# robflynnyh/dynamic-asr-eval

Hardware: AMD Instinct MI355X
Metric: audio-sec/s dynamic-eval (fwd+1 adapt step) (higher is better)
Workload: dtype f32; 1 GPU; run_dynamic_eval_full: 1 h Earnings-22-shape recording per step (360000 frames, seq_len 16384, overlap 14336, offline, MADGRAD lr 9e-05, 6 freq masks <=34), SCConformerXL 6x768 V+1=4096 seeded weights; windows_per_recording=169, chains_per_gpu=2, lockstep_group=4, hip_graphs=True, pcie_inclusive=False

## Files before the change

dynamic-asr-eval_amd/csrc/gemm_f32.hip:

```cpp
#include <algorithm>
#include "common.h"
#include <cstdlib>

typedef float f32x16 __attribute__((ext_vector_type(16)));

namespace {

#ifndef DYN_GEMM_BK
#define DYN_GEMM_BK 32
#endif
constexpr int BK = DYN_GEMM_BK;
constexpr int LDK = BK + 4;
constexpr int KV = BK / 4;
constexpr int RP = 256 / KV;
constexpr int NTHREADS = 256;

struct KParams {
    int64_t M, N, K;
    const float* A; int64_t lda, sa1, sa2;
    const float* B; int64_t ldb, sb1, sb2;
    float* C; int64_t ldc, sc1, sc2;
    int64_t cin_delta;
    const float* bias;
    int64_t bs1, bs2;
// ... 4 lines not shown
    float* ws;
    int64_t nbatch;
    int tiles_n;
    int tiles_m;
    int n_major;
    int64_t tiles_per_batch;
    int64_t full_items;
    int tail_f;
    float* tail_ws;
    int epi;
    float* aux;
    int* counters;
    float* colsum;
    float colsum_beta;
    int64_t first_item;
};

__device__ __forceinline__ float epi_value(float alpha, float acc, float beta, const float* cin, float bias) {
    float v = __fmul_rn(alpha, acc);
    if (beta != 0.f) v = __fmaf_rn(beta, *cin, v);
    return __fadd_rn(v, bias);
}

__device__ __forceinline__ float silu_f(float v) { return v * dyn::sigmoidf_(v); }
__device__ __forceinline__ float silu_grad_f(float u) {
    const float sg = dyn::sigmoidf_(u);
    return sg * (1.f + u * (1.f - sg));
}

template <bool KMAJOR, int R>
__device__ __forceinline__ void load_tile_full(const float* __restrict__ base, int64_t ld, int64_t row0, int64_t k0,
                                               float4 (&reg)[(R * BK / 1024)]) {
    const int t = threadIdx.x;
    if (KMAJOR) {
        const float* p = base + (row0 + (t / KV)) * ld + k0 + 4 * (t % KV);
#pragma unroll
        for (int j = 0; j < (R * BK / 1024); ++j) reg[j] = *reinterpret_cast<const float4*>(p + (int64_t)(RP * j) * ld);
    } else {
        constexpr int RV = R / 4;
        constexpr int KSTEP = NTHREADS / RV;
        const float* p = base + (k0 + t / RV) * ld + row0 + 4 * (t % RV);
#pragma unroll
        for (int j = 0; j < (R * BK / 1024); ++j) reg[j] = *reinterpret_cast<const float4*>(p + (int64_t)(KSTEP * j) * ld);
    }
}

// ... 107 lines not shown
        }
        step = KMAJOR ? (int64_t)BK : (int64_t)BK * ld;
    }
    __device__ __forceinline__ void issue(float* tile, int wave) {
#pragma unroll
        for (int j = 0; j < NI; ++j) {
            __builtin_amdgcn_global_load_lds((gbl_void_t*)ptr[j], (lds_void_t*)(tile + (wave * NI + j) * 256), 16, 0, 0);
            ptr[j] += step;
        }
    }
};

template <bool KMAJOR, int R>
__device__ __forceinline__ void read_frag_glds(const float* __restrict__ s, int roff, int i, int h, int c, float (&f)[4]) {
    if (KMAJOR) {
        const float4 v = *reinterpret_cast<const float4*>(&s[(roff + i) * BK + 4 * ((2 * c + h) ^ ((i >> 1) & 7))]);
        f[0] = v.x; f[1] = v.y; f[2] = v.z; f[3] = v.w;
    } else {
#pragma unroll
        for (int q = 0; q < 4; ++q) f[q] = s[(8 * c + 4 * h + q) * R + roff + i];
    }
}

template <bool TA, bool TB, int BM, int BN, bool VEC, bool GLDS, bool GROUPED, int NW = 4>
__device__ __forceinline__ void gemm_tile(const KParams& p, const int64_t bid, float* smem) {
    constexpr bool AK = !TA;
    constexpr bool BKM = TB;
    constexpr int WM = NW / 2;
    constexpr int WTM = BM / (32 * WM), WTN = BN / 64;
    static_assert(NW == 4 || (NW == 8 && GLDS), "the 8-wave tile exists for direct-to-LDS staging only");
    static_assert(!GLDS || (VEC && BK == 32), "direct-to-LDS staging needs 16-B aligned operands and BK = 32");
    constexpr int SA = GLDS ? BM * BK : BM * LDK, SB = GLDS ? BN * BK : BN * LDK;

    const bool is_tail = !GROUPED && bid >= p.full_items;
    int64_t item;
    int sub = 0;
    if (GROUPED) {
        item = bid;
    } else if (!is_tail) {
        const int64_t nwg = p.full_items;
        const int64_t xcd = bid & 7, q = nwg >> 3, r = nwg & 7;
        item = (xcd < r ? xcd * (q + 1) : r * (q + 1) + (xcd - r) * q) + (bid >> 3);
    } else {
        const int64_t t = bid - p.full_items;
        item = p.full_items + t / p.tail_f;
        sub = (int)(t % p.tail_f);
    }
    const int ks = (int)(item % p.splits);
    const int64_t t2 = item / p.splits;
    const int tile = (int)(t2 % p.tiles_per_batch);
    const int zb = (int)(t2 / p.tiles_per_batch);
    const int tm = p.n_major ? tile % p.tiles_m : tile / p.tiles_n;
    const int tn = p.n_major ? tile / p.tiles_m : tile % p.tiles_n;
    const int64_t z1 = zb / p.nb2, z2 = zb % p.nb2;
    const float* A = p.A + z1 * p.sa1 + z2 * p.sa2;
    const float* B = p.B + z1 * p.sb1 + z2 * p.sb2;

    const int64_t m0 = (int64_t)tm * BM, n0 = (int64_t)tn * BN;
    int64_t kbeg = (int64_t)ks * p.kchunk;
    int64_t kend = (kbeg + p.kchunk < p.K) ? kbeg + p.kchunk : p.K;
    if (is_tail) {
        const int64_t kt_all = (kend - kbeg + BK - 1) / BK;
        const int64_t per = (kt_all + p.tail_f - 1) / p.tail_f;
        const int64_t kb2 = kbeg + (int64_t)sub * per * BK;
        const int64_t ke2 = kb2 + per * BK;
        kend = ke2 < kend ? ke2 : kend;
        kbeg = kb2;
    }
    const int nk = kend > kbeg ? (int)((kend - kbeg + BK - 1) / BK) : 0;

    const int lane = threadIdx.x & 63, wave = threadIdx.x >> 6;
    const int i = lane & 31, h = lane >> 5;
    const int wm = wave >> 1, wn = wave & 1;

    f32x16 acc[WTM][WTN];
#pragma unroll
    for (int a = 0; a < WTM; ++a)
#pragma unroll
        for (int b = 0; b < WTN; ++b)
#pragma unroll
            for (int e = 0; e < 16; ++e) acc[a][b][e] = 0.f;

    float4 ra[BM * BK / 1024], rb[BN * BK / 1024];
    const bool interior = VEC && (m0 + BM <= p.M) && (n0 + BN <= p.N);
    auto fetch = [&](int64_t k0) {
        if (interior && k0 + BK <= kend) {
            load_tile_full<AK, BM>(A, p.lda, m0, k0, ra);
            load_tile_full<BKM, BN>(B, p.ldb, n0, k0, rb);
        } else {
            load_tile<AK, BM, VEC>(A, p.lda, m0, p.M, k0, kend, ra);
            load_tile<BKM, BN, VEC>(B, p.ldb, n0, p.N, k0, kend, rb);
        }
    };
    GldsStager<AK, BM, NW> stA;
    GldsStager<BKM, BN, NW> stB;
    if (GLDS) {
        stA.init(A, p.lda, m0, p.M, kbeg, wave, lane);
        stB.init(B, p.ldb, n0, p.N, kbeg, wave, lane);
        if (nk > 0) { stA.issue(smem, wave); stB.issue(smem + SA, wave); }
    } else if (nk > 0) {
        fetch(kbeg);
        store_tile<AK, BM>(smem, ra);
        store_tile<BKM, BN>(smem + SA, rb);
    }
    if (GLDS) asm volatile("s_waitcnt vmcnt(0)" ::: "memory");
    __syncthreads();

    constexpr int NC = BK / 8;
    constexpr int NREADS = (AK ? WTM : 4 * WTM) + (BKM ? WTN : 4 * WTN);
    static_assert(NC % 2 == 0, "the register ping-pong assumes an even number of k-chunks per tile");
    float fa[2][WTM][4], fb[2][WTN][4];
    auto read_chunk = [&](const float* sa, const float* sb, int c, int slot) {
#pragma unroll
        for (int a = 0; a < WTM; ++a) {
            if (GLDS) read_frag_glds<AK, BM>(sa, wm * (BM / WM) + a * 32, i, h, c, fa[slot][a]);
            else read_frag<AK, BM>(sa, wm * (BM / WM) + a * 32, i, h, c, fa[slot][a]);
        }
#pragma unroll
        for (int b = 0; b < WTN; ++b) {
            if (GLDS) read_frag_glds<BKM, BN>(sb, wn * (BN / 2) + b * 32, i, h, c, fb[slot][b]);
            else read_frag<BKM, BN>(sb, wn * (BN / 2) + b * 32, i, h, c, fb[slot][b]);
        }
    };
    float csum[WTM];
#pragma unroll
    for (int a = 0; a < WTM; ++a) csum[a] = 0.f;
    const bool do_colsum = GROUPED && p.colsum != nullptr && tn == 0 && wn == 0;
    auto mfma_chunk = [&](int slot) {
        if (GROUPED && do_colsum) {
#pragma unroll
            for (int a = 0; a < WTM; ++a) csum[a] += (fa[slot][a][0] + fa[slot][a][1]) + (fa[slot][a][2] + fa[slot][a][3]);
        }
#pragma unroll
        for (int s = 0; s < 4; ++s)
#pragma unroll
            for (int a = 0; a < WTM; ++a)
#pragma unroll
                for (int b = 0; b < WTN; ++b)
                    acc[a][b] = __builtin_amdgcn_mfma_f32_32x32x2f32(fa[slot][a][s], fb[slot][b][s], acc[a][b], 0, 0, 0);
    };
    int cur = 0;
    if (nk > 0) read_chunk(smem, smem + SA, 0, 0);
    for (int kt = 0; kt < nk; ++kt) {
        const float* sa = smem + cur * (SA + SB);
// ... 9 lines not shown
        for (int c = 0; c < NC - 1; ++c) {
            read_chunk(sa, sb, c + 1, (c + 1) & 1);
            mfma_chunk(c & 1);
            __builtin_amdgcn_sched_group_barrier(0x100, NREADS, 0);
            __builtin_amdgcn_sched_group_barrier(0x008, 4 * WTM * WTN, 0);
        }
        if (!GLDS && more) {
            store_tile<AK, BM>(da, ra);
            store_tile<BKM, BN>(da + SA, rb);
        }
        if (GLDS) asm volatile("s_waitcnt vmcnt(0)" ::: "memory");
        __syncthreads();
        if (more) read_chunk(da, da + SA, 0, 0);
        mfma_chunk((NC - 1) & 1);
        __builtin_amdgcn_sched_group_barrier(0x100, NREADS, 0);
        __builtin_amdgcn_sched_group_barrier(0x008, 4 * WTM * WTN, 0);
        cur ^= 1;
    }

    if (GROUPED && do_colsum) {
#pragma unroll
        for (int a = 0; a < WTM; ++a) {
            const float tot = csum[a] + __shfl_xor(csum[a], 32);
            const int64_t m = m0 + wm * (BM / WM) + a * 32 + i;
            if (h == 0 && m < p.M) p.colsum[m] = (p.colsum_beta != 0.f ? p.colsum_beta * p.colsum[m] : 0.f) + tot;
        }
    }
    const bool partial = !GROUPED && (is_tail || p.splits > 1);
    if (partial && p.counters == nullptr) {
        if (is_tail) {
            float* W = p.tail_ws + ((item - p.full_items) * p.tail_f + sub) * (int64_t)(BM * BN);
#pragma unroll
            for (int a = 0; a < WTM; ++a)
#pragma unroll
                for (int b = 0; b < WTN; ++b) {
                    float* wp = W + (wm * (BM / WM) + a * 32 + 4 * h) * BN + wn * (BN / 2) + b * 32 + i;
#pragma unroll
                    for (int e = 0; e < 16; ++e) wp[((e & 3) + 8 * (e >> 2)) * BN] = acc[a][b][e];
                }
        } else {
            float* W = p.ws + ((int64_t)ks * p.nbatch + zb) * p.M * p.N;
#pragma unroll
            for (int a = 0; a < WTM; ++a)
#pragma unroll
                for (int b = 0; b < WTN; ++b) {
                    const int64_t col = n0 + wn * (BN / 2) + b * 32 + i;
#pragma unroll
                    for (int e = 0; e < 16; ++e) {
                        const int64_t row = m0 + wm * (BM / WM) + a * 32 + (e & 3) + 8 * (e >> 2) + 4 * h;
                        if (row < p.M && col < p.N) W[row * p.N + col] = acc[a][b][e];
                    }
                }
        }
        return;
    }
    if (partial) {
        const int64_t pt = is_tail ? (item - p.full_items) : t2;
        const int sl = is_tail ? sub : ks;
        const int nsl = is_tail ? p.tail_f : p.splits;
        float* W0 = p.tail_ws + pt * nsl * (int64_t)(BM * BN);
        float* W = W0 + (int64_t)sl * (BM * BN);
#pragma unroll
        for (int a = 0; a < WTM; ++a)
#pragma unroll
            for (int b = 0; b < WTN; ++b) {
                float* wp = W + (wm * (BM / WM) + a * 32 + 4 * h) * BN + wn * (BN / 2) + b * 32 + i;
#pragma unroll
                for (int e = 0; e < 16; ++e) wp[((e & 3) + 8 * (e >> 2)) * BN] = acc[a][b][e];
            }
        __threadfence();
        __syncthreads();
        int* flag = reinterpret_cast<int*>(smem);
        if (threadIdx.x == 0) flag[0] = (atomicAdd(&p.counters[pt], 1) == nsl - 1) ? 1 : 0;
        __syncthreads();
        if (flag[0] == 0) return;
        __threadfence();
#pragma unroll
        for (int a = 0; a < WTM; ++a)
#pragma unroll
            for (int b = 0; b < WTN; ++b) {
                const float* rp = W0 + (wm * (BM / WM) + a * 32 + 4 * h) * BN + wn * (BN / 2) + b * 32 + i;
#pragma unroll
                for (int e = 0; e < 16; ++e) {
                    const float* q = rp + ((e & 3) + 8 * (e >> 2)) * BN;
                    float t = q[0];
                    for (int k = 1; k < nsl; ++k) t += q[(int64_t)k * (BM * BN)];
                    acc[a][b][e] = t;
                }
            }
        if (threadIdx.x == 0) p.counters[pt] = 0;
    }
    if (m0 + BM <= p.M && n0 + BN <= p.N) {
        float* C = p.C + z1 * p.sc1 + z2 * p.sc2;
#pragma unroll
        for (int a = 0; a < WTM; ++a)
#pragma unroll
            for (int b = 0; b < WTN; ++b) {
                const int64_t col = n0 + wn * (BN / 2) + b * 32 + i;
                const float bv = p.bias ? p.bias[z1 * p.bs1 + z2 * p.bs2 + col] : 0.f;
                float* cp = C + (m0 + wm * (BM / WM) + a * 32 + 4 * h) * p.ldc + col;
                if (p.epi != 0) {
                    const int64_t ad = p.aux - p.C;
#pragma unroll
                    for (int e = 0; e < 16; ++e) {
                        float* q2 = cp + (int64_t)((e & 3) + 8 * (e >> 2)) * p.ldc;
                        const float v = epi_value(p.alpha, acc[a][b][e], p.beta, q2 + p.cin_delta, bv);
                        if (p.epi == 1) { if (p.aux) q2[ad] = v; *q2 = silu_f(v); }
                        else *q2 = v * silu_grad_f(q2[ad]);
                    }
                } else if (p.beta != 0.f) {
#pragma unroll
                    for (int e = 0; e < 16; ++e) {
                        float* q2 = cp + (int64_t)((e & 3) + 8 * (e >> 2)) * p.ldc;
                        *q2 = epi_value(p.alpha, acc[a][b][e], p.beta, q2 + p.cin_delta, bv);
                    }
                } else {
#pragma unroll
                    for (int e = 0; e < 16; ++e) cp[(int64_t)((e & 3) + 8 * (e >> 2)) * p.ldc] = epi_value(p.alpha, acc[a][b][e], 0.f, nullptr, bv);
                }
            }
    } else {
        float* C = p.C + z1 * p.sc1 + z2 * p.sc2;
#pragma unroll
        for (int a = 0; a < WTM; ++a)
#pragma unroll
            for (int b = 0; b < WTN; ++b) {
                const int64_t col = n0 + wn * (BN / 2) + b * 32 + i;
                const float bv = (p.bias && col < p.N) ? p.bias[z1 * p.bs1 + z2 * p.bs2 + col] : 0.f;
#pragma unroll
                for (int e = 0; e < 16; ++e) {
                    const int64_t row = m0 + wm * (BM / WM) + a * 32 + (e & 3) + 8 * (e >> 2) + 4 * h;
                    if (row < p.M && col < p.N) {
                        float v = epi_value(p.alpha, acc[a][b][e], p.beta, C + row * p.ldc + col + p.cin_delta, bv);
                        if (p.epi == 1) { if (p.aux) C[row * p.ldc + col + (p.aux - p.C)] = v; v = silu_f(v); }
                        else if (p.epi == 2) v *= silu_grad_f(C[row * p.ldc + col + (p.aux - p.C)]);
                        C[row * p.ldc + col] = v;
                    }
                }
            }
    }
}

#ifndef DYN_GEMM_WAVES_PER_EU
#define DYN_GEMM_WAVES_PER_EU 2
#endif
template <bool TA, bool TB, int BM, int BN, bool VEC, bool GLDS, int NW = 4>
__global__ __launch_bounds__(NW * 64) __attribute__((amdgpu_waves_per_eu(DYN_GEMM_WAVES_PER_EU, 8))) void gemm_f32_kernel(const KParams p) {
    constexpr int SA = GLDS ? BM * BK : BM * LDK, SB = GLDS ? BN * BK : BN * LDK;
    __shared__ __attribute__((aligned(16))) float smem[2 * (SA + SB)];
    gemm_tile<TA, TB, BM, BN, VEC, GLDS, false, NW>(p, (int64_t)blockIdx.x, smem);
}

constexpr int kMaxGroups = 96;
constexpr int kTableChunk = 12;
struct KTableChunk { KParams g[kTableChunk]; };

__global__ void gemm_table_kernel(const KTableChunk chunk, KParams* __restrict__ table, int base, int count) {
    const int t = threadIdx.x;
    if (t < count) table[base + t] = chunk.g[t];
}

template <bool TA, bool TB, int BM, int BN, bool GLDS>
__global__ __launch_bounds__(NTHREADS) void gemm_f32_grouped_kernel(const KParams* __restrict__ table, int n_groups, int64_t total_items) {
    constexpr int SA = GLDS ? BM * BK : BM * LDK, SB = GLDS ? BN * BK : BN * LDK;
    __shared__ __attribute__((aligned(16))) float smem[2 * (SA + SB)];
    const int64_t bid = blockIdx.x;
    const int64_t xcd = bid & 7, q = total_items >> 3, r = total_items & 7;
    const int64_t item = (xcd < r ? xcd * (q + 1) : r * (q + 1) + (xcd - r) * q) + (bid >> 3);
    int lo = 0, hi = n_groups - 1;
    while (lo < hi) {
        const int mid = (lo + hi + 1) >> 1;
        if (table[mid].first_item <= item) lo = mid; else hi = mid - 1;
    }
    const int g = __builtin_amdgcn_readfirstlane(lo);
    const KParams p = table[g];
    gemm_tile<TA, TB, BM, BN, true, GLDS, true>(p, item - p.first_item, smem);
}

__global__ void splitk_reduce_kernel(const KParams p) {
    const int64_t mn = p.M * p.N;
    const int64_t total = mn * p.nbatch;
    for (int64_t idx = (int64_t)blockIdx.x * blockDim.x + threadIdx.x; idx < total;
         idx += (int64_t)gridDim.x * blockDim.x) {
        const int64_t zb = idx / mn, rem = idx % mn;
        const int64_t row = rem / p.N, col = rem % p.N;
        float s = 0.f;
        for (int k = 0; k < p.splits; ++k) s += p.ws[((int64_t)k * p.nbatch + zb) * mn + rem];
        const int64_t z1 = zb / p.nb2, z2 = zb % p.nb2;
        float* C = p.C + z1 * p.sc1 + z2 * p.sc2 + row * p.ldc + col;
        float v = epi_value(p.alpha, s, p.beta, C + p.cin_delta, p.bias ? p.bias[z1 * p.bs1 + z2 * p.bs2 + col] : 0.f);
        if (p.epi == 1) { if (p.aux) C[p.aux - p.C] = v; v = silu_f(v); }
        else if (p.epi == 2) v *= silu_grad_f(C[p.aux - p.C]);
        *C = v;
    }
}

__global__ __launch_bounds__(256) void tail_reduce_kernel(const KParams p, int BM, int BN, int64_t tail_items) {
    const int per_tile = BM * BN / 4;
    const int64_t total = tail_items * per_tile;
// ... 21 lines not shown
            const int64_t col = col0 + j;
            if (col < p.N) {
                float o = epi_value(p.alpha, v[j], p.beta, C + col + p.cin_delta, p.bias ? p.bias[z1 * p.bs1 + z2 * p.bs2 + col] : 0.f);
                if (p.epi == 1) { if (p.aux) C[col + (p.aux - p.C)] = o; o = silu_f(o); }
                else if (p.epi == 2) o *= silu_grad_f(C[col + (p.aux - p.C)]);
                C[col] = o;
            }
        }
    }
}

struct Plan {
    int bm, bn, splits;
    int64_t kchunk;
    int64_t ws_bytes;
    int64_t full_items;
    int64_t tail_items;
    int tail_f;
    int64_t tail_ws_bytes;
};

double tile_eff(int bm, int bn) { return bm == 256 ? 0.84 : (bm == 128 && bn == 128) ? 0.80 : (bm == 64 && bn == 64) ? 0.62 : 0.72; }
int tile_occ(int bm, int bn) { return bm == 256 ? 1 : (bm == 64 && bn == 64) ? 4 : (bm == 128 && bn == 128) ? 2 : 3; }

bool glds_eligible(const dyn_gemm_desc* d) {
    auto al16 = [](const void* q) { return (((uintptr_t)q) & 15) == 0; };
    const bool vec = al16(d->A) && al16(d->B) && (d->lda % 4 == 0) && (d->ldb % 4 == 0) && (d->sa1 % 4 == 0) && (d->sa2 % 4 == 0) &&
                     (d->sb1 % 4 == 0) && (d->sb2 % 4 == 0);
    static const bool allow_glds = [] { const char* e = getenv("DYN_GEMM_GLDS"); return !e || atoi(e) != 0; }();
    const bool ta = d->trans_a != 0, tb = d->trans_b != 0;
    return allow_glds && vec && d->K % BK == 0 && d->K > 0 && (!ta || d->M % 4 == 0) && (tb || d->N % 4 == 0) && (!ta || d->M >= 4) && (tb || d->N >= 4);
}

bool eval_config(const dyn_gemm_desc* d, int bm, int bn, int s, int f_req, Plan* out, double* cost) {
    const int64_t batch = d->nb1 * d->nb2;
    const int64_t ktiles = dyn::cdiv(d->K > 0 ? d->K : 1, BK);
    if (s < 1) s = 1;
    if (s > ktiles) s = (int)ktiles;
    const int64_t tiles = dyn::cdiv(d->M, bm) * dyn::cdiv(d->N, bn);
    const int64_t slots = (int64_t)tile_occ(bm, bn) * 256;
    const int64_t kchunk = dyn::cdiv(ktiles, s) * BK;
    const int s_eff = (int)dyn::cdiv(d->K > 0 ? d->K : 1, kchunk);
    const int64_t items = tiles * batch * s_eff;
    const int64_t rounds = items / slots, rem = items % slots;
    int f = 1;
    if (s_eff == 1 && rem > 0 && f_req != 1) {
// ... 58 lines not shown
            return best;
        }
    }
    const int cand[4][2] = {{128, 128}, {128, 64}, {64, 128}, {64, 64}};
    int split_opts[9] = {1, 2, 3, 4, 6, 8, 12, 16, 24};
    int n_opts = 9;
    if (d->split_k > 0) { split_opts[0] = d->split_k; n_opts = 1; }
    double best_cost = 1e300;
    for (int c = 0; c < 4; ++c) {
        const int bm = cand[c][0], bn = cand[c][1];
        if ((d->M <= 64 && bm == 128) || (d->N <= 64 && bn == 128)) continue;
        for (int so = 0; so < n_opts; ++so) {
            const int s = split_opts[so];
            if (d->split_k == 0 && s > 1 && (d->K / s < 256)) continue;
            Plan pl;
            eval_config(d, bm, bn, s, d->split_k == 0 ? -1 : 1, &pl, &cost);
            if (cost < best_cost) { best_cost = cost; best = pl; }
        }
    }
    return best;
}

template <bool TA, bool TB, int BM, int BN>
void launch_vec(const KParams& kp, bool vec, dim3 grid, hipStream_t st) {
    static const bool allow_glds = [] { const char* e = getenv("DYN_GEMM_GLDS"); return !e || atoi(e) != 0; }();
    const bool glds = allow_glds && vec && kp.K % BK == 0 && kp.K > 0 && (!TA || kp.M % 4 == 0) && (TB || kp.N % 4 == 0) &&
                      (!TA || kp.M >= 4) && (TB || kp.N >= 4);
    if (glds) hipLaunchKernelGGL((gemm_f32_kernel<TA, TB, BM, BN, true, true>), grid, dim3(NTHREADS), 0, st, kp);
    else if (vec) hipLaunchKernelGGL((gemm_f32_kernel<TA, TB, BM, BN, true, false>), grid, dim3(NTHREADS), 0, st, kp);
    else hipLaunchKernelGGL((gemm_f32_kernel<TA, TB, BM, BN, false, false>), grid, dim3(NTHREADS), 0, st, kp);
}

template <bool TA, bool TB>
void launch_tile(const KParams& kp, const Plan& pl, bool vec, dim3 grid, hipStream_t st) {
    if (pl.bm == 256) hipLaunchKernelGGL((gemm_f32_kernel<TA, TB, 256, 128, true, true, 8>), grid, dim3(512), 0, st, kp);
    else if (pl.bm == 128 && pl.bn == 128) launch_vec<TA, TB, 128, 128>(kp, vec, grid, st);
    else if (pl.bm == 128 && pl.bn == 64) launch_vec<TA, TB, 128, 64>(kp, vec, grid, st);
    else if (pl.bm == 64 && pl.bn == 128) launch_vec<TA, TB, 64, 128>(kp, vec, grid, st);
    else launch_vec<TA, TB, 64, 64>(kp, vec, grid, st);
}

}

extern "C" int64_t dyn_gemm_f32_workspace_bytes(const dyn_gemm_desc* d) {
    if (!d || d->M <= 0 || d->N <= 0 || d->nb1 <= 0 || d->nb2 <= 0) return 0;
    const Plan pl = make_plan(d);
    return pl.ws_bytes > pl.tail_ws_bytes ? pl.ws_bytes : pl.tail_ws_bytes;
}

extern "C" int dyn_gemm_f32(const dyn_gemm_desc* d, void* stream) {
    DYN_REQUIRE(d != nullptr, DYN_E_ARG, "dyn_gemm_f32: null descriptor");
    DYN_REQUIRE(d->M >= 0 && d->N >= 0 && d->K >= 0 && d->nb1 >= 1 && d->nb2 >= 1, DYN_E_ARG,
                "dyn_gemm_f32: bad sizes M=%lld N=%lld K=%lld nb=%lldx%lld", (long long)d->M, (long long)d->N,
                (long long)d->K, (long long)d->nb1, (long long)d->nb2);
    if (d->M == 0 || d->N == 0) return DYN_OK;
    DYN_REQUIRE(d->A && d->B && d->C, DYN_E_ARG, "dyn_gemm_f32: null operand");
    DYN_REQUIRE(d->epilogue >= 0 && d->epilogue <= 2 && (d->epilogue != 2 || d->aux), DYN_E_ARG,
                "dyn_gemm_f32: epilogue %d needs 0 <= mode <= 2 (and aux for mode 2)", d->epilogue);
    DYN_REQUIRE(d->a_colsum == nullptr, DYN_E_ARG, "dyn_gemm_f32: a_colsum is a grouped-launch feature (dyn_gemm_f32_grouped)");
    DYN_REQUIRE(d->lda >= (d->trans_a ? d->M : 1) && d->ldb >= (d->trans_b ? d->K : 1) && d->ldc >= d->N,
                DYN_E_ARG, "dyn_gemm_f32: leading dimension smaller than the row length");
    Plan pl = make_plan(d);
// ... 15 lines not shown
    kp.bias = d->bias; kp.bs1 = d->bias_s1; kp.bs2 = d->bias_s2; kp.alpha = d->alpha; kp.beta = d->beta;
    kp.cin_delta = d->C_in ? (int64_t)(d->C_in - d->C) : 0;
    kp.nb2 = d->nb2; kp.splits = pl.splits; kp.kchunk = pl.kchunk;
    kp.ws = (float*)d->workspace; kp.nbatch = batch;
    const int64_t tiles_m = dyn::cdiv(d->M, pl.bm), tiles_n = dyn::cdiv(d->N, pl.bn);
    kp.tiles_n = (int)tiles_n;
    kp.tiles_m = (int)tiles_m;
    static const bool xcd_map = [] { const char* e = getenv("DYN_GEMM_XCDMAP"); return !e || atoi(e) != 0; }();
    kp.n_major = (xcd_map && d->N > d->M) ? 1 : 0;
    kp.tiles_per_batch = tiles_m * tiles_n;
    kp.full_items = pl.full_items;
    kp.tail_f = pl.tail_f;
    kp.tail_ws = (float*)d->workspace;
    kp.epi = d->epilogue; kp.aux = d->aux;
    const int64_t n_ptiles = pl.splits > 1 ? tiles_m * tiles_n * batch : pl.tail_items;
    kp.counters = (d->counters && n_ptiles > 0 && n_ptiles <= d->n_counters) ? d->counters : nullptr;
    kp.colsum = nullptr; kp.colsum_beta = 0.f; kp.first_item = 0;
    const int64_t nblocks = pl.full_items + pl.tail_items * pl.tail_f;
    DYN_REQUIRE(nblocks < (1ll << 31) && tiles_m * tiles_n < (1ll << 31), DYN_E_ARG, "dyn_gemm_f32: grid too large (%lld workgroups)",
                (long long)nblocks);
    auto al16 = [](const void* q) { return (((uintptr_t)q) & 15) == 0; };
    const bool vec = al16(d->A) && al16(d->B) && (d->lda % 4 == 0) && (d->ldb % 4 == 0) && (d->sa1 % 4 == 0) &&
                     (d->sa2 % 4 == 0) && (d->sb1 % 4 == 0) && (d->sb2 % 4 == 0);
    dim3 grid((unsigned)nblocks);
    hipStream_t st = (hipStream_t)stream;
    if (!d->trans_a && !d->trans_b) launch_tile<false, false>(kp, pl, vec, grid, st);
    else if (!d->trans_a && d->trans_b) launch_tile<false, true>(kp, pl, vec, grid, st);
    else if (d->trans_a && !d->trans_b) launch_tile<true, false>(kp, pl, vec, grid, st);
    else launch_tile<true, true>(kp, pl, vec, grid, st);
    int rc = dyn::check_launch("dyn_gemm_f32");
    if (rc != DYN_OK) return rc;
    if (kp.counters != nullptr) return rc;
    if (pl.splits > 1) {
        const int64_t total = d->M * d->N * batch;
        int64_t nblk = dyn::cdiv(total, 256);
        if (nblk > 2048) nblk = 2048;
        hipLaunchKernelGGL(splitk_reduce_kernel, dim3((unsigned)nblk), dim3(256), 0, st, kp);
        rc = dyn::check_launch("dyn_gemm_f32(splitk_reduce)");
    } else if (pl.tail_items > 0) {
        int64_t nblk = dyn::cdiv(pl.tail_items * pl.bm * pl.bn / 4, 256);
        if (nblk > 4096) nblk = 4096;
        hipLaunchKernelGGL(tail_reduce_kernel, dim3((unsigned)nblk), dim3(256), 0, st, kp, pl.bm, pl.bn, pl.tail_items);
        rc = dyn::check_launch("dyn_gemm_f32(tail_reduce)");
    }
    return rc;
}

extern "C" int64_t dyn_gemm_f32_grouped_workspace_bytes(int32_t n) {
    return (int64_t)(n > 0 ? n : 0) * (int64_t)sizeof(KParams);
}

extern "C" int dyn_gemm_f32_grouped(const dyn_gemm_desc* descs, int32_t n, void* workspace, int64_t workspace_bytes, void* stream) {
    DYN_REQUIRE(descs != nullptr && n >= 0 && n <= kMaxGroups, DYN_E_ARG, "dyn_gemm_f32_grouped: need 0 <= n <= %d descriptors", kMaxGroups);
    if (n == 0) return DYN_OK;
    DYN_REQUIRE(workspace && workspace_bytes >= dyn_gemm_f32_grouped_workspace_bytes(n), DYN_E_WORKSPACE,
                "dyn_gemm_f32_grouped: workspace %lld < %lld bytes", (long long)workspace_bytes,
                (long long)dyn_gemm_f32_grouped_workspace_bytes(n));
    const bool ta = descs[0].trans_a != 0, tb = descs[0].trans_b != 0;
    constexpr int BM = 128, BN = 128;
    auto al16 = [](const void* q) { return (((uintptr_t)q) & 15) == 0; };
    bool glds = true;
    KParams host[kMaxGroups];
    int64_t total = 0;
    int used = 0;
    for (int g = 0; g < n; ++g) {
        const dyn_gemm_desc* d = &descs[g];
        DYN_REQUIRE((d->trans_a != 0) == ta && (d->trans_b != 0) == tb, DYN_E_ARG, "dyn_gemm_f32_grouped: group %d has other transpose flags", g);
        DYN_REQUIRE(d->nb1 == 1 && d->nb2 == 1 && d->split_k == 0 && d->epilogue == 0 && d->bias == nullptr, DYN_E_ARG,
                    "dyn_gemm_f32_grouped: group %d: batches, split-K, bias and activation epilogues are not supported here", g);
        DYN_REQUIRE(d->M >= 0 && d->N >= 0 && d->K >= 0, DYN_E_ARG, "dyn_gemm_f32_grouped: group %d has a negative size", g);
        if (d->M == 0 || d->N == 0) continue;
        DYN_REQUIRE(d->A && d->B && d->C, DYN_E_ARG, "dyn_gemm_f32_grouped: group %d has a null operand", g);
        DYN_REQUIRE(d->lda >= (ta ? d->M : d->K) && d->ldb >= (tb ? d->K : d->N) && d->ldc >= d->N, DYN_E_ARG,
                    "dyn_gemm_f32_grouped: group %d: leading dimension smaller than the row length", g);
        DYN_REQUIRE(al16(d->A) && al16(d->B) && d->lda % 4 == 0 && d->ldb % 4 == 0, DYN_E_ARG,
                    "dyn_gemm_f32_grouped: group %d: operands must be 16-byte aligned with leading dimensions that are multiples of 4", g);
        DYN_REQUIRE(d->a_colsum == nullptr || ta, DYN_E_ARG, "dyn_gemm_f32_grouped: a_colsum needs trans_a (A stored [K][M])");
        glds = glds && d->K % BK == 0 && d->K > 0 && (!ta || (d->M % 4 == 0 && d->M >= 4)) && (tb || (d->N % 4 == 0 && d->N >= 4));
        KParams& kp = host[used++];
        kp.M = d->M; kp.N = d->N; kp.K = d->K;
        kp.A = d->A; kp.lda = d->lda; kp.sa1 = 0; kp.sa2 = 0;
        kp.B = d->B; kp.ldb = d->ldb; kp.sb1 = 0; kp.sb2 = 0;
        kp.C = d->C; kp.ldc = d->ldc; kp.sc1 = 0; kp.sc2 = 0;
        kp.cin_delta = d->C_in ? (int64_t)(d->C_in - d->C) : 0;
        kp.bias = nullptr; kp.bs1 = 0; kp.bs2 = 0; kp.alpha = d->alpha; kp.beta = d->beta;
        kp.nb2 = 1; kp.splits = 1; kp.kchunk = dyn::cdiv(d->K > 0 ? d->K : 1, BK) * BK;
        kp.ws = nullptr; kp.nbatch = 1;
        kp.tiles_m = (int)dyn::cdiv(d->M, BM); kp.tiles_n = (int)dyn::cdiv(d->N, BN);
        kp.n_major = 0;
        kp.tiles_per_batch = (int64_t)kp.tiles_m * kp.tiles_n;
        kp.full_items = kp.tiles_per_batch; kp.tail_f = 1; kp.tail_ws = nullptr;
        kp.epi = 0; kp.aux = nullptr; kp.counters = nullptr;
        kp.colsum = d->a_colsum; kp.colsum_beta = d->a_colsum_beta;
        kp.first_item = total;
        total += kp.tiles_per_batch;
    }
    if (used == 0) return DYN_OK;
    DYN_REQUIRE(total < (1ll << 31), DYN_E_ARG, "dyn_gemm_f32_grouped: grid too large");
    static const bool allow_glds = [] { const char* e = getenv("DYN_GEMM_GLDS"); return !e || atoi(e) != 0; }();
    glds = glds && allow_glds;
    hipStream_t st = (hipStream_t)stream;
    KParams* table = (KParams*)workspace;
    for (int base = 0; base < used; base += kTableChunk) {
        KTableChunk chunk;
        const int cnt = used - base < kTableChunk ? used - base : kTableChunk;
        for (int t = 0; t < cnt; ++t) chunk.g[t] = host[base + t];
        for (int t = cnt; t < kTableChunk; ++t) chunk.g[t] = host[base];
        hipLaunchKernelGGL(gemm_table_kernel, dim3(1), dim3(64), 0, st, chunk, table, base, cnt);
    }
    dim3 grid((unsigned)total);
#define GO_G(TA_, TB_)                                                                                                              \
    do {                                                                                                                            \
        if (glds) hipLaunchKernelGGL((gemm_f32_grouped_kernel<TA_, TB_, BM, BN, true>), grid, dim3(NTHREADS), 0, st, table, used, total); \
        else hipLaunchKernelGGL((gemm_f32_grouped_kernel<TA_, TB_, BM, BN, false>), grid, dim3(NTHREADS), 0, st, table, used, total);     \
    } while (0)
    if (ta && !tb) GO_G(true, false);
    else if (!ta && tb) GO_G(false, true);
    else if (!ta && !tb) GO_G(false, false);
    else GO_G(true, true);
#undef GO_G
    return dyn::check_launch("dyn_gemm_f32_grouped");
}
```

include/dyneval.h:

```cpp
#ifndef DYNEVAL_H_
#define DYNEVAL_H_
#include <stdint.h>

#ifdef __cplusplus
extern "C" {
#endif

#define DYN_OK 0
#define DYN_E_ARG (-1)
#define DYN_E_LAUNCH (-2)
#define DYN_E_WORKSPACE (-3)
#define DYN_E_UNSUPPORTED (-4)

const char* dyn_last_error(void);
const char* dyn_version(void);
const char* dyn_arch(void);

typedef struct {
    int32_t trans_a, trans_b;
    int64_t M, N, K;
    float alpha, beta;
    const float* A; int64_t lda, sa1, sa2;
    const float* B; int64_t ldb, sb1, sb2;
    float* C;       int64_t ldc, sc1, sc2;
    const float* bias;
    int64_t nb1, nb2;
    int32_t split_k;
    void* workspace; int64_t workspace_bytes;
    int32_t tile_m, tile_n, tail_slices, reserved_;
    const float* C_in;
    int32_t epilogue, reserved2_;
    float* aux;
    float* a_colsum;
    float a_colsum_beta, reserved3_;
    int32_t* counters;
    int64_t n_counters;
    int64_t bias_s1, bias_s2;
} dyn_gemm_desc;

int64_t dyn_gemm_f32_workspace_bytes(const dyn_gemm_desc* d);
int dyn_gemm_f32(const dyn_gemm_desc* d, void* stream);
int64_t dyn_gemm_f32_grouped_workspace_bytes(int32_t n);
int dyn_gemm_f32_grouped(const dyn_gemm_desc* descs, int32_t n, void* workspace, int64_t workspace_bytes, void* stream);

int dyn_gemm_bf16x3_nt(const float* X, const float* W, const float* bias, float* C, int64_t M, int64_t N, int64_t K, int64_t ldx,
                       int64_t ldw, int64_t ldc, void* stream);
int dyn_gemm_bf16x3(int trans_a, int trans_b, const float* A, const float* B, const float* bias, float* C, int64_t M, int64_t N, int64_t K,
                    int64_t lda, int64_t ldb, int64_t ldc, void* stream);
int dyn_bf16x3_split(const float* src, void* planes, int64_t rows, int64_t K, int64_t ld, void* stream);
int dyn_gemm_bf16x3_presplit(const float* X, const void* w_planes, const float* bias, float* C, int64_t M, int64_t N, int64_t K, int64_t ldx,
                             int64_t ldc, void* stream);

int dyn_silu_fwd(const float* x, float* y, int64_t n, void* stream);
int dyn_silu_bwd(const float* x, const float* dy, float* dx, int64_t n, void* stream);
int dyn_glu_fwd(const float* u, float* y, int64_t rows, int64_t C, void* stream);
int dyn_glu_bwd(const float* u, const float* dy, float* du, int64_t rows, int64_t C, void* stream);
int dyn_axpby(const float* x, float* y, float a, float b, int64_t n, void* stream);
int64_t dyn_colsum_workspace_bytes(int64_t rows, int64_t C);
int dyn_colsum(const float* x, float* out, int64_t rows, int64_t C, float beta, void* workspace, int64_t workspace_bytes,
               void* stream);
int dyn_reduce_partials(const float* partial, float* out, int64_t P, int64_t n, float beta, void* stream);
int dyn_reduce_defer_begin(void* arena, int64_t arena_bytes);
int dyn_reduce_defer_flush(void* stream);
int dyn_reduce_defer_abort(void);
int dyn_transpose_ft(const float* x, float* y, int64_t F, int64_t T, int64_t ldx, void* stream);

// ... 229 lines not shown
```

Before: 791.6 audio-s/s.

## Interleave MFMA block rows/cols so row-contiguous LDS reads and C stores use float2

Adds a WIDE variant of the f32 GEMM tile. When a wave owns two 32-wide blocks along a row-contiguous operand dimension (TA for A, !TB for B), the two blocks are interleaved element-wise. That lets one float2 LDS read fill both fragments instead of scalar reads, and lets the epilogue write C (and aux/C_in/bias) as float2 pairs. The aim is fewer LDS instructions in the inner loop and fewer global store transactions. The cost is more template instantiations and an 8-byte alignment requirement checked at launch. It is on by default and can be turned off with an env var or an API call.

```diff
diff --git a/dynamic-asr-eval_amd/csrc/gemm_f32.hip b/dynamic-asr-eval_amd/csrc/gemm_f32.hip
--- a/dynamic-asr-eval_amd/csrc/gemm_f32.hip
+++ b/dynamic-asr-eval_amd/csrc/gemm_f32.hip
@@ -50,6 +50,12 @@
     return __fadd_rn(v, bias);
 }
 
+__device__ __forceinline__ float epi_value_v(float alpha, float acc, float beta, float cin, float bias) {
+    float v = __fmul_rn(alpha, acc);
+    if (beta != 0.f) v = __fmaf_rn(beta, cin, v);
+    return __fadd_rn(v, bias);
+}
+
 __device__ __forceinline__ float silu_f(float v) { return v * dyn::sigmoidf_(v); }
 __device__ __forceinline__ float silu_grad_f(float u) {
     const float sg = dyn::sigmoidf_(u);
@@ -203,12 +209,28 @@
     }
 }
 
-template <bool TA, bool TB, int BM, int BN, bool VEC, bool GLDS, bool GROUPED, int NW = 4>
+template <int LD>
+__device__ __forceinline__ void read_frag_pair(const float* __restrict__ s, int roff, int i, int h, int c, float (&f0)[4], float (&f1)[4]) {
+    const float* p = s + (8 * c + 4 * h) * LD + roff + 2 * i;
+#pragma unroll
+    for (int q = 0; q < 4; ++q) {
+        const float2 v = *reinterpret_cast<const float2*>(p + q * LD);
+        f0[q] = v.x; f1[q] = v.y;
+    }
+}
+
+template <bool TA, bool TB, int BM, int BN, int NW>
+constexpr bool has_row_pairs() { return (TA && BM / (32 * (NW / 2)) == 2) || (!TB && BN / 64 == 2); }
+
+template <bool TA, bool TB, int BM, int BN, bool VEC, bool GLDS, bool GROUPED, int NW = 4, bool WIDE = false>
 __device__ __forceinline__ void gemm_tile(const KParams& p, const int64_t bid, float* smem) {
     constexpr bool AK = !TA;
     constexpr bool BKM = TB;
     constexpr int WM = NW / 2;
     constexpr int WTM = BM / (32 * WM), WTN = BN / 64;
+    constexpr bool PA = WIDE && TA && WTM == 2;
+    constexpr bool PB = WIDE && !TB && WTN == 2;
+    static_assert(!WIDE || PA || PB, "WIDE is instantiated only where a row-contiguous operand has two blocks per wave");
     static_assert(NW == 4 || (NW == 8 && GLDS), "the 8-wave tile exists for direct-to-LDS staging only");
     static_assert(!GLDS || (VEC && BK == 32), "direct-to-LDS staging needs 16-B aligned operands and BK = 32");
     constexpr int SA = GLDS ? BM * BK : BM * LDK, SB = GLDS ? BN * BK : BN * LDK;
@@ -253,6 +275,9 @@
     const int lane = threadIdx.x & 63, wave = threadIdx.x >> 6;
     const int i = lane & 31, h = lane >> 5;
     const int wm = wave >> 1, wn = wave & 1;
+    auto trow = [&](int a, int r) { return wm * (BM / WM) + (PA ? 2 * r + a : a * 32 + r); };
+    auto tcol = [&](int b, int c) { return wn * (BN / 2) + (PB ? 2 * c + b : b * 32 + c); };
+    constexpr int RS = PA ? 2 : 1;
 
     f32x16 acc[WTM][WTN];
 #pragma unroll
@@ -288,19 +313,27 @@
     __syncthreads();
 
     constexpr int NC = BK / 8;
-    constexpr int NREADS = (AK ? WTM : 4 * WTM) + (BKM ? WTN : 4 * WTN);
+    constexpr int NREADS = (AK ? WTM : PA ? 2 : 4 * WTM) + (BKM ? WTN : PB ? 2 : 4 * WTN);
     static_assert(NC % 2 == 0, "the register ping-pong assumes an even number of k-chunks per tile");
     float fa[2][WTM][4], fb[2][WTN][4];
     auto read_chunk = [&](const float* sa, const float* sb, int c, int slot) {
-#pragma unroll
-        for (int a = 0; a < WTM; ++a) {
-            if (GLDS) read_frag_glds<AK, BM>(sa, wm * (BM / WM) + a * 32, i, h, c, fa[slot][a]);
-            else read_frag<AK, BM>(sa, wm * (BM / WM) + a * 32, i, h, c, fa[slot][a]);
-        }
-#pragma unroll
-        for (int b = 0; b < WTN; ++b) {
-            if (GLDS) read_frag_glds<BKM, BN>(sb, wn * (BN / 2) + b * 32, i, h, c, fb[slot][b]);
-            else read_frag<BKM, BN>(sb, wn * (BN / 2) + b * 32, i, h, c, fb[slot][b]);
+        if constexpr (PA) {
+            read_frag_pair<GLDS ? BM : BM + 4>(sa, wm * (BM / WM), i, h, c, fa[slot][0], fa[slot][1]);
+        } else {
+#pragma unroll
+            for (int a = 0; a < WTM; ++a) {
+                if (GLDS) read_frag_glds<AK, BM>(sa, wm * (BM / WM) + a * 32, i, h, c, fa[slot][a]);
+                else read_frag<AK, BM>(sa, wm * (BM / WM) + a * 32, i, h, c, fa[slot][a]);
+            }
+        }
+        if constexpr (PB) {
+            read_frag_pair<GLDS ? BN : BN + 4>(sb, wn * (BN / 2), i, h, c, fb[slot][0], fb[slot][1]);
+        } else {
+#pragma unroll
+            for (int b = 0; b < WTN; ++b) {
+                if (GLDS) read_frag_glds<BKM, BN>(sb, wn * (BN / 2) + b * 32, i, h, c, fb[slot][b]);
+                else read_frag<BKM, BN>(sb, wn * (BN / 2) + b * 32, i, h, c, fb[slot][b]);
+            }
         }
     };
     float csum[WTM];
@@ -356,7 +389,7 @@
 #pragma unroll
         for (int a = 0; a < WTM; ++a) {
             const float tot = csum[a] + __shfl_xor(csum[a], 32);
-            const int64_t m = m0 + wm * (BM / WM) + a * 32 + i;
+            const int64_t m = m0 + trow(a, i);
             if (h == 0 && m < p.M) p.colsum[m] = (p.colsum_beta != 0.f ? p.colsum_beta * p.colsum[m] : 0.f) + tot;
         }
     }
@@ -368,9 +401,9 @@
             for (int a = 0; a < WTM; ++a)
 #pragma unroll
                 for (int b = 0; b < WTN; ++b) {
-                    float* wp = W + (wm * (BM / WM) + a * 32 + 4 * h) * BN + wn * (BN / 2) + b * 32 + i;
-#pragma unroll
-                    for (int e = 0; e < 16; ++e) wp[((e & 3) + 8 * (e >> 2)) * BN] = acc[a][b][e];
+                    float* wp = W + trow(a, 4 * h) * BN + tcol(b, i);
+#pragma unroll
+                    for (int e = 0; e < 16; ++e) wp[RS * ((e & 3) + 8 * (e >> 2)) * BN] = acc[a][b][e];
                 }
         } else {
             float* W = p.ws + ((int64_t)ks * p.nbatch + zb) * p.M * p.N;
@@ -378,10 +411,10 @@
             for (int a = 0; a < WTM; ++a)
 #pragma unroll
                 for (int b = 0; b < WTN; ++b) {
-                    const int64_t col = n0 + wn * (BN / 2) + b * 32 + i;
+                    const int64_t col = n0 + tcol(b, i);
 #pragma unroll
                     for (int e = 0; e < 16; ++e) {
-                        const int64_t row = m0 + wm * (BM / WM) + a * 32 + (e & 3) + 8 * (e >> 2) + 4 * h;
+                        const int64_t row = m0 + trow(a, (e & 3) + 8 * (e >> 2) + 4 * h);
                         if (row < p.M && col < p.N) W[row * p.N + col] = acc[a][b][e];
                     }
                 }
@@ -398,9 +431,9 @@
         for (int a = 0; a < WTM; ++a)
 #pragma unroll
             for (int b = 0; b < WTN; ++b) {
-                float* wp = W + (wm * (BM / WM) + a * 32 + 4 * h) * BN + wn * (BN / 2) + b * 32 + i;
-#pragma unroll
-                for (int e = 0; e < 16; ++e) wp[((e & 3) + 8 * (e >> 2)) * BN] = acc[a][b][e];
+                float* wp = W + trow(a, 4 * h) * BN + tcol(b, i);
+#pragma unroll
+                for (int e = 0; e < 16; ++e) wp[RS * ((e & 3) + 8 * (e >> 2)) * BN] = acc[a][b][e];
             }
         __threadfence();
         __syncthreads();
@@ -413,10 +446,10 @@
         for (int a = 0; a < WTM; ++a)
 #pragma unroll
             for (int b = 0; b < WTN; ++b) {
-                const float* rp = W0 + (wm * (BM / WM) + a * 32 + 4 * h) * BN + wn * (BN / 2) + b * 32 + i;
+                const float* rp = W0 + trow(a, 4 * h) * BN + tcol(b, i);
 #pragma unroll
                 for (int e = 0; e < 16; ++e) {
-                    const float* q = rp + ((e & 3) + 8 * (e >> 2)) * BN;
+                    const float* q = rp + RS * ((e & 3) + 8 * (e >> 2)) * BN;
                     float t = q[0];
                     for (int k = 1; k < nsl; ++k) t += q[(int64_t)k * (BM * BN)];
                     acc[a][b][e] = t;
@@ -426,44 +459,79 @@
     }
     if (m0 + BM <= p.M && n0 + BN <= p.N) {
         float* C = p.C + z1 * p.sc1 + z2 * p.sc2;
-#pragma unroll
-        for (int a = 0; a < WTM; ++a)
-#pragma unroll
-            for (int b = 0; b < WTN; ++b) {
-                const int64_t col = n0 + wn * (BN / 2) + b * 32 + i;
-                const float bv = p.bias ? p.bias[z1 * p.bs1 + z2 * p.bs2 + col] : 0.f;
-                float* cp = C + (m0 + wm * (BM / WM) + a * 32 + 4 * h) * p.ldc + col;
+        if constexpr (PB) {
+            auto ld2 = [](const float* q) { return *reinterpret_cast<const float2*>(q); };
+            auto st2 = [](float* q, float x, float y) { *reinterpret_cast<float2*>(q) = make_float2(x, y); };
+            const int64_t col = n0 + tcol(0, i);
+            const float2 bv = p.bias ? ld2(p.bias + z1 * p.bs1 + z2 * p.bs2 + col) : make_float2(0.f, 0.f);
+#pragma unroll
+            for (int a = 0; a < WTM; ++a) {
+                float* cp = C + (m0 + trow(a, 4 * h)) * p.ldc + col;
                 if (p.epi != 0) {
                     const int64_t ad = p.aux - p.C;
 #pragma unroll
                     for (int e = 0; e < 16; ++e) {
-                        float* q2 = cp + (int64_t)((e & 3) + 8 * (e >> 2)) * p.ldc;
-                        const float v = epi_value(p.alpha, acc[a][b][e], p.beta, q2 + p.cin_delta, bv);
-                        if (p.epi == 1) { if (p.aux) q2[ad] = v; *q2 = silu_f(v); }
-                        else *q2 = v * silu_grad_f(q2[ad]);
+                        float* q2 = cp + (int64_t)(RS * ((e & 3) + 8 * (e >> 2))) * p.ldc;
+                        const float2 ci = p.beta != 0.f ? ld2(q2 + p.cin_delta) : make_float2(0.f, 0.f);
+                        const float v0 = epi_value_v(p.alpha, acc[a][0][e], p.beta, ci.x, bv.x);
+                        const float v1 = epi_value_v(p.alpha, acc[a][1][e], p.beta, ci.y, bv.y);
+                        if (p.epi == 1) { if (p.aux) st2(q2 + ad, v0, v1); st2(q2, silu_f(v0), silu_f(v1)); }
+                        else { const float2 u = ld2(q2 + ad); st2(q2, v0 * silu_grad_f(u.x), v1 * silu_grad_f(u.y)); }
                     }
                 } else if (p.beta != 0.f) {
 #pragma unroll
                     for (int e = 0; e < 16; ++e) {
-                        float* q2 = cp + (int64_t)((e & 3) + 8 * (e >> 2)) * p.ldc;
-                        *q2 = epi_value(p.alpha, acc[a][b][e], p.beta, q2 + p.cin_delta, bv);
+                        float* q2 = cp + (int64_t)(RS * ((e & 3) + 8 * (e >> 2))) * p.ldc;
+                        const float2 ci = ld2(q2 + p.cin_delta);
+                        st2(q2, epi_value_v(p.alpha, acc[a][0][e], p.beta, ci.x, bv.x), epi_value_v(p.alpha, acc[a][1][e], p.beta, ci.y, bv.y));
                     }
                 } else {
 #pragma unroll
-                    for (int e = 0; e < 16; ++e) cp[(int64_t)((e & 3) + 8 * (e >> 2)) * p.ldc] = epi_value(p.alpha, acc[a][b][e], 0.f, nullptr, bv);
+                    for (int e = 0; e < 16; ++e)
+                        st2(cp + (int64_t)(RS * ((e & 3) + 8 * (e >> 2))) * p.ldc, epi_value_v(p.alpha, acc[a][0][e], 0.f, 0.f, bv.x),
+                            epi_value_v(p.alpha, acc[a][1][e], 0.f, 0.f, bv.y));
                 }
             }
+        } else {
+#pragma unroll
+            for (int a = 0; a < WTM; ++a)
+#pragma unroll
+                for (int b = 0; b < WTN; ++b) {
+                    const int64_t col = n0 + tcol(b, i);
+                    const float bv = p.bias ? p.bias[z1 * p.bs1 + z2 * p.bs2 + col] : 0.f;
+                    float* cp = C + (m0 + trow(a, 4 * h)) * p.ldc + col;
+                    if (p.epi != 0) {
+                        const int64_t ad = p.aux - p.C;
+#pragma unroll
+                        for (int e = 0; e < 16; ++e) {
+                            float* q2 = cp + (int64_t)(RS * ((e & 3) + 8 * (e >> 2))) * p.ldc;
+                            const float v = epi_value(p.alpha, acc[a][b][e], p.beta, q2 + p.cin_delta, bv);
+                            if (p.epi == 1) { if (p.aux) q2[ad] = v; *q2 = silu_f(v); }
+                            else *q2 = v * silu_grad_f(q2[ad]);
+                        }
+                    } else if (p.beta != 0.f) {
+#pragma unroll
+                        for (int e = 0; e < 16; ++e) {
+                            float* q2 = cp + (int64_t)(RS * ((e & 3) + 8 * (e >> 2))) * p.ldc;
+                            *q2 = epi_value(p.alpha, acc[a][b][e], p.beta, q2 + p.cin_delta, bv);
+                        }
+                    } else {
+#pragma unroll
+                        for (int e = 0; e < 16; ++e) cp[(int64_t)(RS * ((e & 3) + 8 * (e >> 2))) * p.ldc] = epi_value(p.alpha, acc[a][b][e], 0.f, nullptr, bv);
+                    }
+                }
+        }
     } else {
         float* C = p.C + z1 * p.sc1 + z2 * p.sc2;
 #pragma unroll
         for (int a = 0; a < WTM; ++a)
 #pragma unroll
             for (int b = 0; b < WTN; ++b) {
-                const int64_t col = n0 + wn * (BN / 2) + b * 32 + i;
+                const int64_t col = n0 + tcol(b, i);
                 const float bv = (p.bias && col < p.N) ? p.bias[z1 * p.bs1 + z2 * p.bs2 + col] : 0.f;
 #pragma unroll
                 for (int e = 0; e < 16; ++e) {
-                    const int64_t row = m0 + wm * (BM / WM) + a * 32 + (e & 3) + 8 * (e >> 2) + 4 * h;
+                    const int64_t row = m0 + trow(a, (e & 3) + 8 * (e >> 2) + 4 * h);
                     if (row < p.M && col < p.N) {
                         float v = epi_value(p.alpha, acc[a][b][e], p.beta, C + row * p.ldc + col + p.cin_delta, bv);
                         if (p.epi == 1) { if (p.aux) C[row * p.ldc + col + (p.aux - p.C)] = v; v = silu_f(v); }
@@ -478,11 +546,11 @@
 #ifndef DYN_GEMM_WAVES_PER_EU
 #define DYN_GEMM_WAVES_PER_EU 2
 #endif
-template <bool TA, bool TB, int BM, int BN, bool VEC, bool GLDS, int NW = 4>
+template <bool TA, bool TB, int BM, int BN, bool VEC, bool GLDS, int NW = 4, bool WIDE = false>
 __global__ __launch_bounds__(NW * 64) __attribute__((amdgpu_waves_per_eu(DYN_GEMM_WAVES_PER_EU, 8))) void gemm_f32_kernel(const KParams p) {
     constexpr int SA = GLDS ? BM * BK : BM * LDK, SB = GLDS ? BN * BK : BN * LDK;
     __shared__ __attribute__((aligned(16))) float smem[2 * (SA + SB)];
-    gemm_tile<TA, TB, BM, BN, VEC, GLDS, false, NW>(p, (int64_t)blockIdx.x, smem);
+    gemm_tile<TA, TB, BM, BN, VEC, GLDS, false, NW, WIDE>(p, (int64_t)blockIdx.x, smem);
 }
 
 constexpr int kMaxGroups = 96;
@@ -494,7 +562,7 @@
     if (t < count) table[base + t] = chunk.g[t];
 }
 
-template <bool TA, bool TB, int BM, int BN, bool GLDS>
+template <bool TA, bool TB, int BM, int BN, bool GLDS, bool WIDE = false>
 __global__ __launch_bounds__(NTHREADS) void gemm_f32_grouped_kernel(const KParams* __restrict__ table, int n_groups, int64_t total_items) {
     constexpr int SA = GLDS ? BM * BK : BM * LDK, SB = GLDS ? BN * BK : BN * LDK;
     __shared__ __attribute__((aligned(16))) float smem[2 * (SA + SB)];
@@ -508,7 +576,7 @@
     }
     const int g = __builtin_amdgcn_readfirstlane(lo);
     const KParams p = table[g];
-    gemm_tile<TA, TB, BM, BN, true, GLDS, true>(p, item - p.first_item, smem);
+    gemm_tile<TA, TB, BM, BN, true, GLDS, true, 4, WIDE>(p, item - p.first_item, smem);
 }
 
 __global__ void splitk_reduce_kernel(const KParams p) {
@@ -576,6 +644,15 @@
 
 double tile_eff(int bm, int bn) { return bm == 256 ? 0.84 : (bm == 128 && bn == 128) ? 0.80 : (bm == 64 && bn == 64) ? 0.62 : 0.72; }
 int tile_occ(int bm, int bn) { return bm == 256 ? 1 : (bm == 64 && bn == 64) ? 4 : (bm == 128 && bn == 128) ? 2 : 3; }
+
+int g_wide_t = [] { const char* e = getenv("DYN_GEMM_WIDE_T"); return (!e || atoi(e) != 0) ? 1 : 0; }();
+
+bool wide_ok(const float* C, int64_t ldc, int64_t sc1, int64_t sc2, const float* C_in, const float* aux, const float* bias,
+             int64_t bs1, int64_t bs2) {
+    auto al8 = [](const void* q) { return (((uintptr_t)q) & 7) == 0; };
+    return g_wide_t != 0 && al8(C) && ldc % 2 == 0 && sc1 % 2 == 0 && sc2 % 2 == 0 && (!C_in || al8(C_in)) && (!aux || al8(aux)) &&
+           (!bias || (al8(bias) && bs1 % 2 == 0 && bs2 % 2 == 0));
+}
 
 bool glds_eligible(const dyn_gemm_desc* d) {
     auto al16 = [](const void* q) { return (((uintptr_t)q) & 15) == 0; };
@@ -680,22 +757,31 @@
 }
 
 template <bool TA, bool TB, int BM, int BN>
-void launch_vec(const KParams& kp, bool vec, dim3 grid, hipStream_t st) {
+void launch_vec(const KParams& kp, bool vec, bool wide, dim3 grid, hipStream_t st) {
     static const bool allow_glds = [] { const char* e = getenv("DYN_GEMM_GLDS"); return !e || atoi(e) != 0; }();
     const bool glds = allow_glds && vec && kp.K % BK == 0 && kp.K > 0 && (!TA || kp.M % 4 == 0) && (TB || kp.N % 4 == 0) &&
                       (!TA || kp.M >= 4) && (TB || kp.N >= 4);
+    if constexpr (has_row_pairs<TA, TB, BM, BN, 4>()) {
+        if (wide && glds) { hipLaunchKernelGGL((gemm_f32_kernel<TA, TB, BM, BN, true, true, 4, true>), grid, dim3(NTHREADS), 0, st, kp); return; }
+        if (wide && vec) { hipLaunchKernelGGL((gemm_f32_kernel<TA, TB, BM, BN, true, false, 4, true>), grid, dim3(NTHREADS), 0, st, kp); return; }
+    }
     if (glds) hipLaunchKernelGGL((gemm_f32_kernel<TA, TB, BM, BN, true, true>), grid, dim3(NTHREADS), 0, st, kp);
     else if (vec) hipLaunchKernelGGL((gemm_f32_kernel<TA, TB, BM, BN, true, false>), grid, dim3(NTHREADS), 0, st, kp);
     else hipLaunchKernelGGL((gemm_f32_kernel<TA, TB, BM, BN, false, false>), grid, dim3(NTHREADS), 0, st, kp);
 }
 
 template <bool TA, bool TB>
-void launch_tile(const KParams& kp, const Plan& pl, bool vec, dim3 grid, hipStream_t st) {
-    if (pl.bm == 256) hipLaunchKernelGGL((gemm_f32_kernel<TA, TB, 256, 128, true, true, 8>), grid, dim3(512), 0, st, kp);
-    else if (pl.bm == 128 && pl.bn == 128) launch_vec<TA, TB, 128, 128>(kp, vec, grid, st);
-    else if (pl.bm == 128 && pl.bn == 64) launch_vec<TA, TB, 128, 64>(kp, vec, grid, st);
-    else if (pl.bm == 64 && pl.bn == 128) launch_vec<TA, TB, 64, 128>(kp, vec, grid, st);
-    else launch_vec<TA, TB, 64, 64>(kp, vec, grid, st);
+void launch_tile(const KParams& kp, const Plan& pl, bool vec, bool wide, dim3 grid, hipStream_t st) {
+    if (pl.bm == 256) {
+        if constexpr (has_row_pairs<TA, TB, 256, 128, 8>()) {
+            if (wide) { hipLaunchKernelGGL((gemm_f32_kernel<TA, TB, 256, 128, true, true, 8, true>), grid, dim3(512), 0, st, kp); return; }
+        }
+        hipLaunchKernelGGL((gemm_f32_kernel<TA, TB, 256, 128, true, true, 8>), grid, dim3(512), 0, st, kp);
+    }
+    else if (pl.bm == 128 && pl.bn == 128) launch_vec<TA, TB, 128, 128>(kp, vec, wide, grid, st);
+    else if (pl.bm == 128 && pl.bn == 64) launch_vec<TA, TB, 128, 64>(kp, vec, wide, grid, st);
+    else if (pl.bm == 64 && pl.bn == 128) launch_vec<TA, TB, 64, 128>(kp, vec, wide, grid, st);
+    else launch_vec<TA, TB, 64, 64>(kp, vec, wide, grid, st);
 }
 
 }
@@ -757,12 +843,13 @@
     auto al16 = [](const void* q) { return (((uintptr_t)q) & 15) == 0; };
     const bool vec = al16(d->A) && al16(d->B) && (d->lda % 4 == 0) && (d->ldb % 4 == 0) && (d->sa1 % 4 == 0) &&
                      (d->sa2 % 4 == 0) && (d->sb1 % 4 == 0) && (d->sb2 % 4 == 0);
+    const bool wide = wide_ok(d->C, d->ldc, d->sc1, d->sc2, d->C_in, d->aux, d->bias, d->bias_s1, d->bias_s2);
     dim3 grid((unsigned)nblocks);
     hipStream_t st = (hipStream_t)stream;
-    if (!d->trans_a && !d->trans_b) launch_tile<false, false>(kp, pl, vec, grid, st);
-    else if (!d->trans_a && d->trans_b) launch_tile<false, true>(kp, pl, vec, grid, st);
-    else if (d->trans_a && !d->trans_b) launch_tile<true, false>(kp, pl, vec, grid, st);
-    else launch_tile<true, true>(kp, pl, vec, grid, st);
+    if (!d->trans_a && !d->trans_b) launch_tile<false, false>(kp, pl, vec, wide, grid, st);
+    else if (!d->trans_a && d->trans_b) launch_tile<false, true>(kp, pl, vec, wide, grid, st);
+    else if (d->trans_a && !d->trans_b) launch_tile<true, false>(kp, pl, vec, wide, grid, st);
+    else launch_tile<true, true>(kp, pl, vec, wide, grid, st);
     int rc = dyn::check_launch("dyn_gemm_f32");
     if (rc != DYN_OK) return rc;
     if (kp.counters != nullptr) return rc;
@@ -794,7 +881,7 @@
     const bool ta = descs[0].trans_a != 0, tb = descs[0].trans_b != 0;
     constexpr int BM = 128, BN = 128;
     auto al16 = [](const void* q) { return (((uintptr_t)q) & 15) == 0; };
-    bool glds = true;
+    bool glds = true, wide = true;
     KParams host[kMaxGroups];
     int64_t total = 0;
     int used = 0;
@@ -812,6 +899,7 @@
                     "dyn_gemm_f32_grouped: group %d: operands must be 16-byte aligned with leading dimensions that are multiples of 4", g);
         DYN_REQUIRE(d->a_colsum == nullptr || ta, DYN_E_ARG, "dyn_gemm_f32_grouped: a_colsum needs trans_a (A stored [K][M])");
         glds = glds && d->K % BK == 0 && d->K > 0 && (!ta || (d->M % 4 == 0 && d->M >= 4)) && (tb || (d->N % 4 == 0 && d->N >= 4));
+        wide = wide && wide_ok(d->C, d->ldc, 0, 0, d->C_in, nullptr, nullptr, 0, 0);
         KParams& kp = host[used++];
         kp.M = d->M; kp.N = d->N; kp.K = d->K;
         kp.A = d->A; kp.lda = d->lda; kp.sa1 = 0; kp.sa2 = 0;
@@ -844,15 +932,21 @@
         hipLaunchKernelGGL(gemm_table_kernel, dim3(1), dim3(64), 0, st, chunk, table, base, cnt);
     }
     dim3 grid((unsigned)total);
-#define GO_G(TA_, TB_)                                                                                                              \
-    do {                                                                                                                            \
-        if (glds) hipLaunchKernelGGL((gemm_f32_grouped_kernel<TA_, TB_, BM, BN, true>), grid, dim3(NTHREADS), 0, st, table, used, total); \
-        else hipLaunchKernelGGL((gemm_f32_grouped_kernel<TA_, TB_, BM, BN, false>), grid, dim3(NTHREADS), 0, st, table, used, total);     \
+#define GO_G(TA_, TB_, W_)                                                                                                              \
+    do {                                                                                                                                \
+        if (glds) hipLaunchKernelGGL((gemm_f32_grouped_kernel<TA_, TB_, BM, BN, true, W_>), grid, dim3(NTHREADS), 0, st, table, used, total); \
+        else hipLaunchKernelGGL((gemm_f32_grouped_kernel<TA_, TB_, BM, BN, false, W_>), grid, dim3(NTHREADS), 0, st, table, used, total);     \
     } while (0)
-    if (ta && !tb) GO_G(true, false);
-    else if (!ta && tb) GO_G(false, true);
-    else if (!ta && !tb) GO_G(false, false);
-    else GO_G(true, true);
+    if (ta && !tb) { if (wide) GO_G(true, false, true); else GO_G(true, false, false); }
+    else if (!ta && tb) GO_G(false, true, false);
+    else if (!ta && !tb) { if (wide) GO_G(false, false, true); else GO_G(false, false, false); }
+    else { if (wide) GO_G(true, true, true); else GO_G(true, true, false); }
 #undef GO_G
     return dyn::check_launch("dyn_gemm_f32_grouped");
 }
+
+extern "C" int dyn_gemm_set_wide_t(int32_t on) {
+    const int prev = g_wide_t;
+    if (on >= 0) g_wide_t = on != 0 ? 1 : 0;
+    return prev;
+}
diff --git a/include/dyneval.h b/include/dyneval.h
--- a/include/dyneval.h
+++ b/include/dyneval.h
@@ -42,6 +42,7 @@
 int dyn_gemm_f32(const dyn_gemm_desc* d, void* stream);
 int64_t dyn_gemm_f32_grouped_workspace_bytes(int32_t n);
 int dyn_gemm_f32_grouped(const dyn_gemm_desc* descs, int32_t n, void* workspace, int64_t workspace_bytes, void* stream);
+int dyn_gemm_set_wide_t(int32_t on);
 
 int dyn_gemm_bf16x3_nt(const float* X, const float* W, const float* bias, float* C, int64_t M, int64_t N, int64_t K, int64_t ldx,
                        int64_t ldw, int64_t ldc, void* stream);
```

Measured after the change: 790.9 audio-s/s (median of 3 runs). No clear change (-0.1%).
